# CYF2000127/MolNexTR

Hardware: AMD Instinct MI355X
Metric: molecules/sec (384x384, bs32 per GPU), full predict hot path (higher is better)
Workload: dtype fp16x3

## Files before the change

include/molnextr_hip.h:

```cpp
#ifndef MOLNEXTR_HIP_H
#define MOLNEXTR_HIP_H

#include <stddef.h>
#include <stdint.h>

#ifdef __cplusplus
extern "C" {
#endif

#define MNX_ABI_VERSION 7

typedef struct mnx_engine mnx_engine;

typedef enum {
    MNX_OK = 0,
    MNX_ERR_INVALID_ARG = -1,
    MNX_ERR_WEIGHTS = -2,
    MNX_ERR_HIP = -3,
    MNX_ERR_NO_DEVICE = -4,
    MNX_ERR_CAPACITY = -5,
    MNX_ERR_RANGE = -6
} mnx_status;

enum { MNX_DTYPE_BF16 = 0, MNX_DTYPE_FP16 = 1, MNX_DTYPE_FP32 = 2, MNX_DTYPE_BF16X3 = 3, MNX_DTYPE_FP16X3 = 4,
// ... 177 lines not shown
               int32_t N, int32_t K, void* stream);

int mnx_gemm16_split(mnx_engine* h, int32_t epi, const void* A, int64_t a_lo, const void* W, int64_t w_lo, float oscale,
                     void* C, int64_t c_lo, const float* bias, int32_t M, int32_t N, int32_t K, int32_t terms,
                     void* stream);

int mnx_window_attn(mnx_engine* h, const void* qkv, int64_t qkv_lo, const float* table, void* out, int64_t out_lo,
                    int32_t B, int32_t H, int32_t W, int32_t C, int32_t heads, int32_t shift, int32_t terms, void* stream);

int mnx_kv_block(mnx_engine* h, int32_t which, int32_t layer, int32_t owner, int32_t head, void* dst, void* stream);

int mnx_patch_embed(mnx_engine* h, const void* img, int32_t img_format, const float* w_t, const float* bias,
                    const float* gamma, const float* beta, float* x, int32_t B, int32_t S, int32_t C, void* stream);

int mnx_layernorm16(mnx_engine* h, const float* x, const float* gamma, const float* beta, void* y16, int64_t y_lo,
                    float* y32, int32_t M, int32_t C, float eps, int32_t planes, int32_t* flag, void* stream);
int mnx_merge_ln16(mnx_engine* h, const float* x, const float* gamma, const float* beta, void* y16, int64_t y_lo,
                   int32_t B, int32_t H, int32_t W, int32_t C, float eps, int32_t planes, void* stream);

int mnx_cast16(mnx_engine* h, const float* x, void* y16, int64_t y_lo, int64_t n, float scale, void* stream);

int mnx_sgemm_tn(mnx_engine* h, const float* A, const float* W, const float* bias, float* C, int32_t M, int32_t N,
                 int32_t K, int32_t perm_S, void* stream);

int mnx_profile_enable(mnx_engine* h, int32_t enable);
int mnx_profile_read(mnx_engine* h, int32_t kind, double* ms, double* work, int64_t* launches);

int mnx_probe_decode_attn(mnx_engine* h, int32_t rows, int32_t t, int32_t iters, double* self_ms, double* cross_ms,
                          void* stream);

int mnx_gemm_clock(mnx_engine* h, int32_t reset, double* mhz);
int mnx_probe_mfma(mnx_engine* h, int32_t ms_target, double* tflops, double* mhz, void* stream);

#ifdef __cplusplus
}
#endif
#endif
```

molnextr_amd/csrc/atom_walk.h:

```cpp
#pragma once
#include "dec_types.h"

namespace mnx {

template <typename Emit>
__device__ __forceinline__ int atom_walk(const int* seq, int n, const unsigned char* fl, const TokenClasses* __restrict__ tc,
                                         Emit emit) {
    const int x0 = tc->x0, y0 = tc->y0, lb = tc->lbracket, rb = tc->rbracket;
    const int iC = tc->id_C, il = tc->id_l, iB = tc->id_B, ir = tc->id_r;
    int i = 0, k = 0;
    while (i < n) {
        const int t = seq[i];
        if (t == 2 || t == 0) break;
        if (t >= x0) { ++i; continue; }
        if (!(fl[t] & 2)) { ++i; continue; }
        int j;
        if (t == lb) {
            j = i + 1;
            while (j < n && seq[j] < x0 && (fl[seq[j]] & 1)) {
                ++j;
                if (seq[j - 1] == rb) break;
            }
        } else if (i + 1 < n && ((t == iC && seq[i + 1] == il) || (t == iB && seq[i + 1] == ir))) {
            j = i + 2;
        } else {
            j = i + 1;
        }
        if (j + 2 < n && seq[j] >= x0 && seq[j] < y0 && seq[j + 1] >= y0) {
            emit(k, i, j);
            ++k;
            i = j + 2;
        } else {
            i = j;
        }
    }
    return k;
}

}
```

molnextr_amd/csrc/dec_types.h:

```cpp
#pragma once
#include <hip/hip_runtime.h>
#include <stdint.h>

struct mnx_mol;
struct mnx_atom;
struct mnx_bond;
struct mnx_molfile;
struct mnx_smiles;

namespace mnx {

constexpr int MAX_SLOTS = 4096;
constexpr int BEGIN_THREADS = 1024;
constexpr int ROW_TILE = 32;
constexpr int MAX_DEC_LAYERS = 8;
constexpr int MAX_CHUNKS = 128;
constexpr int MAX_REF_BATCH = 512;
constexpr int CHUNK_TILES = MAX_REF_BATCH / ROW_TILE;

struct DecState {
    int tick;
    int n_active;
    int chunk_alive[MAX_CHUNKS];
    int alive[MAX_SLOTS];
// ... 21 lines not shown
    const float *lnf_g, *lnf_b;
    const float *w1, *b1, *w2, *b2;
    const float *wqkv_t, *wo_t, *wq2_t, *wo2_t, *w1_t, *w2_t;
};

struct DecWeights {
    DecLayerW L[MAX_DEC_LAYERS];
    const float *emb, *pe, *lnF_g, *lnF_b, *wout_t, *bout;
    const float *w_enc, *b_enc;
    const float *w_memkv, *b_memkv;
    const float *edge_w1cat, *edge_b1cat;
    const float *edge_w2, *edge_b2;
    int layers, heads, dff, vocab, vpad, sym_offset, bins, pe_len, enc_dim;
};

struct DecBuffers {
    DecState* st;
    float *x, *q, *ctx, *h;
    float *x2, *part;
    float *fpart;
    int fpart_rows;
    char *self_k, *self_v;
    float *memory;
    float *mem_kv32;
    char *mem_kv;
    int Tq, Sq;
    int* tokens;
    float* logp;
    float* hidden;
    float *edge_g, *edge_uv, *edge_prob;
    int T, S, slots, mem_blocks, kmax;
};

constexpr int MAX_BEAM_IMGS = 256;
constexpr int MAX_BEAM = 8;
constexpr int BEAM_LP_STRIDE = 256;
constexpr int BEAM_ANC_MAX = 512;

struct BeamState {
    int top_fin[MAX_BEAM_IMGS];
    int n_hyps[MAX_BEAM_IMGS];
    int pool_n[MAX_BEAM_IMGS];
    int order[MAX_BEAM_IMGS][MAX_BEAM];
    float pscore[MAX_BEAM_IMGS][MAX_BEAM];
    int plen[MAX_BEAM_IMGS][MAX_BEAM];
    float cum[MAX_BEAM_IMGS * MAX_BEAM];
};

struct BeamBuffers {
    BeamState* bs;
    float* blp;
    int* anc;
    int* ptok;
    float* phid;
    int B, K, n_best, anc_stride;
    int ref_batch;
    int pool_stride;
};

struct TokenClasses {
    unsigned char flags[256];
    int lbracket, rbracket, id_C, id_l, id_B, id_r, x0, y0, vocab;
};

struct VocabText {
    unsigned char len[256];
    unsigned char name[256][8];
};

hipError_t kvq_pack_enqueue(const float* src, char* dst, int n_blocks, int S, int Sq, hipStream_t s);
constexpr int GUIDE_MASK = 4;
struct GuideRows {
    int* table;
    int stride;
    const int* src;
    int L, n;
};
hipError_t dec_enqueue_admit(const DecBuffers& b, const int* slots_dev, const int* rowc_dev, int n, int chunk_tag,
                             int mem_blk0, int max_len, int stop_on_eos, hipStream_t s, const GuideRows* g = nullptr);
hipError_t dec_enqueue_reset(const DecBuffers& b, hipStream_t s);
hipError_t dec_enqueue_status(const DecBuffers& b, int slots, hipStream_t s);
hipError_t dec_enqueue_tick(const DecWeights& w, const DecBuffers& b, int slots_scan, int rows, float* logits_trace,
                            int trace_rows, hipStream_t s, const BeamBuffers* beam = nullptr, const int* forced = nullptr,
                            int fused_tile = 0, const int* glab = nullptr, int glab_stride = 0);
hipError_t dec_fused_init();
void dec_fused_dump_stamps(const char* path);
hipError_t dec_enqueue_fused_layers(const DecWeights& w, const DecBuffers& b, int rows, int row_tile, hipStream_t s,
                                    const float** x_final, const float** part_final);
hipError_t beam_enqueue_init(const DecBuffers& b, const BeamBuffers& bm, int max_len, hipStream_t s);
hipError_t beam_enqueue_gather(const DecBuffers& b, const BeamBuffers& bm, int out_len, int* o_tokens, int* o_len,
                               float* o_scores, float* o_hidden, hipStream_t s);
hipError_t dec_probe_attn(const DecWeights& w, const DecBuffers& b, int rows, int t, int iters, hipEvent_t* ev,
                          hipStream_t s);
// ... 39 lines not shown
```

molnextr_amd/csrc/decoder.hip:

```cpp
#include <stdlib.h>

#include "common.h"
#include "kernels.h"
#include "dec_types.h"
#include "atom_walk.h"
#include "kvq.h"

namespace mnx {

__global__ __launch_bounds__(256) void sgemm_tn_kernel(const float* __restrict__ A, const float* __restrict__ W,
                                                       const float* __restrict__ bias, float* __restrict__ C, int M,
                                                       int N, int K, int perm_S) {
    __shared__ float As[16][68], Ws[16][68];
    const int tid = threadIdx.x, tx = tid & 15, ty = tid >> 4;
    const int m0 = blockIdx.y * 64, n0 = blockIdx.x * 64;
    const int lr = tid >> 2, lk = (tid & 3) * 4;
    const float* ap = A + (size_t)min(m0 + lr, M - 1) * K + lk;
    const float* wp = W + (size_t)min(n0 + lr, N - 1) * K + lk;
    float acc[4][4] = {};
    f32x4 a = *(const f32x4*)ap, w = *(const f32x4*)wp;
    for (int k0 = 0; k0 < K; k0 += 16) {
#pragma unroll
        for (int j = 0; j < 4; ++j) {
            As[lk + j][lr] = a[j];
            Ws[lk + j][lr] = w[j];
        }
        __syncthreads();
        const int kn = k0 + 16 < K ? k0 + 16 : k0;
// ... 5 lines not shown
#pragma unroll
            for (int i = 0; i < 4; ++i)
#pragma unroll
                for (int j = 0; j < 4; ++j) acc[i][j] = fmaf(av[i], wv[j], acc[i][j]);
        }
        __syncthreads();
    }
    const int n = n0 + tx * 4;
    if (n >= N) return;
    f32x4 b4 = {0.f, 0.f, 0.f, 0.f};
    if (bias) b4 = *(const f32x4*)(bias + n);
#pragma unroll
    for (int i = 0; i < 4; ++i) {
        const int m = m0 + ty * 4 + i;
        if (m < M) {
            const size_t off = perm_S > 0 ? ((((size_t)(m / perm_S) * (N >> 8) + (n >> 8)) * 8 + ((n & 255) >> 5)) * perm_S +
                                             (m % perm_S)) * 32 + (n & 31)
                                          : (size_t)m * N + n;
            *(f32x4*)(C + off) = (f32x4){acc[i][0], acc[i][1], acc[i][2], acc[i][3]} + b4;
        }
    }
}

hipError_t launch_sgemm_tn(const float* A, const float* W, const float* bias, float* C, int M, int N, int K,
                           hipStream_t s, int perm_S) {
    if ((K & 15) || (N & 3) || (perm_S > 0 && ((N & 255) || M % perm_S))) return hipErrorInvalidValue;
    dim3 grid((N + 63) / 64, (M + 63) / 64), block(256);
    hipLaunchKernelGGL(sgemm_tn_kernel, grid, block, 0, s, A, W, bias, C, M, N, K, perm_S);
    return hipGetLastError();
}

__global__ __launch_bounds__(256) void kvq_pack_kernel(const float* __restrict__ src, char* __restrict__ dst, long long n_rows,
                                                       int S, int Sq) {
    const long long r = (long long)blockIdx.x * 32 + (threadIdx.x >> 3);
    const int part = threadIdx.x & 7;
    if (r >= n_rows) return;
    const f32x4 v = *(const f32x4*)(src + r * 32 + part * 4);
    float amax = fmaxf(fmaxf(fabsf(v[0]), fabsf(v[1])), fmaxf(fabsf(v[2]), fabsf(v[3])));
    amax = fmaxf(amax, __shfl_xor(amax, 1, 64));
    amax = fmaxf(amax, __shfl_xor(amax, 2, 64));
    amax = fmaxf(amax, __shfl_xor(amax, 4, 64));
    int q[4];
    float scale = 0.f;
#pragma unroll
    for (int u = 0; u < 4; ++u) kvq_quant(v[u], amax, q[u], scale);
    const long long blk_i = r / S;
    const int key = (int)(r - blk_i * S);
    char* blk = dst + (size_t)blk_i * kvq_block_bytes(Sq);
    kvq_store4(blk, Sq, key, part * 4, q);
    if (part == 0) kvq_store_scale(blk, Sq, key, scale);
}

hipError_t kvq_pack_enqueue(const float* src, char* dst, int n_blocks, int S, int Sq, hipStream_t s) {
    const long long n_rows = (long long)n_blocks * S;
    hipLaunchKernelGGL(kvq_pack_kernel, dim3((unsigned)((n_rows + 31) / 32)), dim3(256), 0, s, src, dst, n_rows, S, Sq);
    return hipGetLastError();
}


constexpr int TN = 32, XS = 260;

struct LinArgs {
    const float* in;
    const float* W;
    const float* bias;
    const float* gamma;
    const float* beta;
    float* out;
    char* kcache;
    char* vcache;
    int Tq;
    float* x_write;
    const float* emb;
    const float* pe;
    const float* part;
    const DecState* st;
    int N, K, T, heads;
    int part_stride;
// ... 498 lines not shown
    h.x = (split_w2 && ((w.layers - 1) & 1)) ? b.x2 : b.x; h.part = split_w2 ? b.part : nullptr; h.part_stride = b.slots * D;
    h.n_part = w.dff / 256;
    if (fused) { h.x = fx; h.part = fp; h.part_stride = b.fpart_rows * D; h.tree_bias = w.L[w.layers - 1].b2; }
    h.gamma = w.lnF_g; h.beta = w.lnF_b; h.wout_t = w.wout_t; h.bout = w.bout; h.st = b.st;
    h.tokens = b.tokens; h.token_logp = b.logp; h.hidden = b.hidden; h.logits_trace = logits_trace;
    h.V = w.vocab; h.VP = w.vpad; h.T = T; h.x0 = w.sym_offset; h.y0 = w.sym_offset + w.bins;
    h.eos = 2; h.trace_rows = trace_rows; h.forced = forced;
    const GuideTab gt{glab, glab_stride};
    if (glab) {
        if (fused) hipLaunchKernelGGL(dec_head4_guided_kernel, dim3(slots), dim3(1024), 0, s, h, gt);
        else hipLaunchKernelGGL(dec_head_guided_kernel, dim3(slots), dim3(256), 0, s, h, gt);
    } else if (beam) {
        h.blp = beam->blp;
        hipLaunchKernelGGL(dec_head_kernel<true>, dim3(slots), dim3(256), 0, s, h);
        hipLaunchKernelGGL(beam_pick_kernel, dim3(beam->B), dim3(256), 0, s, b.st, *beam, b.hidden, b.tokens, T, w.vocab, 2);
    } else if (fused) {
        hipLaunchKernelGGL(dec_head4_kernel, dim3(slots), dim3(1024), 0, s, h);
    } else {
        hipLaunchKernelGGL(dec_head_kernel<false>, dim3(slots), dim3(256), 0, s, h);
    }
    return hipGetLastError();
}

__global__ __launch_bounds__(64) void atom_scan_kernel(const int* __restrict__ lens, const int* __restrict__ tokens,
                                                       const TokenClasses* __restrict__ tc, const int* __restrict__ slots,
                                                       int n_rows, int T, int kmax, int* __restrict__ atom_idx,
                                                       int* __restrict__ n_atoms) {
    __shared__ int seq[512];
    __shared__ unsigned char fl[256];
    const int row = blockIdx.x;
    const int slot = slots ? slots[row] : row;
    const int n = min(lens[slot], 512);
    for (int i = threadIdx.x; i < n; i += 64) seq[i] = tokens[(size_t)slot * T + i];
    for (int i = threadIdx.x; i < 256; i += 64) fl[i] = tc->flags[i];
    __syncthreads();
    if (threadIdx.x != 0) return;
    const int k = atom_walk(seq, n, fl, tc, [&](int a, int, int j) {
        if (a < kmax) atom_idx[(size_t)row * kmax + a] = j + 2;
    });
    n_atoms[row] = k < kmax ? k : kmax;
}

hipError_t atoms_enqueue(const DecBuffers& b, const TokenClasses* tc_dev, const int* slots_dev, int n, int kmax,
                         int* atom_idx, int* n_atoms, hipStream_t s) {
    hipLaunchKernelGGL(atom_scan_kernel, dim3(n), dim3(64), 0, s, b.st->len, b.tokens, tc_dev, slots_dev, n, b.T, kmax,
                       atom_idx, n_atoms);
    return hipGetLastError();
}

hipError_t atoms_enqueue_raw(const TokenClasses* tc_dev, const int* tokens, const int* lens, int n, int T, int kmax,
                             int* atom_idx, int* n_atoms, hipStream_t s) {
    hipLaunchKernelGGL(atom_scan_kernel, dim3(n), dim3(64), 0, s, lens, tokens, tc_dev, (const int*)nullptr, n, T, kmax,
                       atom_idx, n_atoms);
    return hipGetLastError();
}

constexpr int CONF_THREADS = 256;

__global__ __launch_bounds__(CONF_THREADS) void confidence_kernel(
        const int* __restrict__ lens, const int* __restrict__ tokens, const float* __restrict__ logp,
        const TokenClasses* __restrict__ tc, const int* __restrict__ slots, int T, int kmax,
        const int* __restrict__ atom_idx, const int* __restrict__ n_atoms, const double* __restrict__ scores,
        double* __restrict__ atom_scores, double* __restrict__ overall) {
    __shared__ int seq[512];
    __shared__ double ts[512];
    __shared__ unsigned char fl[256];
    __shared__ int span_len[256];
    __shared__ double red_sum[CONF_THREADS], red_prod[CONF_THREADS];
    const int row = blockIdx.x, tid = threadIdx.x;
    const int slot = slots ? slots[row] : row;
    const int n = min(min(lens[slot], T), 512);
    const int k = min(max(n_atoms[row], 0), kmax);
    double sum = 0.0, prod = 1.0;
    for (int i = tid; i < n; i += CONF_THREADS) {
        seq[i] = tokens[(size_t)slot * T + i];
// ... 443 lines not shown
```

molnextr_amd/csrc/engine.hip:

```cpp
#include "../../include/molnextr_hip.h"

#include <hip/hip_runtime.h>

#include <time.h>
#include <cmath>
#include <cstdint>
#include <cstdio>
#include <cstring>
#include <map>
#include <memory>
#include <string>
#include <tuple>
#include <unordered_map>
#include <vector>

#include "dec_types.h"
#include "kernels.h"
#include "kvq.h"

using namespace mnx;

namespace {

thread_local std::string g_create_error;
// ... 516 lines not shown
    if (h->enc_flag && hipMemset(h->enc_flag, 0, sizeof(int)) != hipSuccess) P.problems.push_back("hipMemset failed");
    DecBuffers& db = h->db;
    const int SL = c.dec_slots > 0 ? c.dec_slots : 2048;
    h->n_chunk_bufs = SL / ROW_TILE;
    db.T = c.max_len; db.S = (int)S; db.slots = SL; db.mem_blocks = h->n_chunk_bufs * ROW_TILE; db.kmax = c.max_atoms;
    db.st = (DecState*)P.dalloc(sizeof(DecState));
    db.x = (float*)P.dalloc((size_t)SL * D * 4);
    db.x2 = (float*)P.dalloc((size_t)SL * D * 4);
    db.part = (float*)P.dalloc((size_t)(FF / 256) * SL * D * 4);
    db.fpart_rows = std::min(SL, std::max(ROW_TILE, (std::max(h->dec_fused_max, h->dec_mid_max) + ROW_TILE - 1) / ROW_TILE * ROW_TILE));
    db.fpart = (float*)P.dalloc((size_t)2 * 16 * db.fpart_rows * D * 4);
    if (db.fpart && hipMemset(db.fpart, 0, (size_t)2 * 16 * db.fpart_rows * D * 4) != hipSuccess) P.problems.push_back("hipMemset failed");
    if (dec_fused_init() != hipSuccess) P.problems.push_back("dec_fused_init: LDS opt-in failed");
    db.q = (float*)P.dalloc((size_t)SL * D * 4);
    db.ctx = (float*)P.dalloc((size_t)SL * D * 4);
    db.h = (float*)P.dalloc((size_t)SL * FF * 4);
    db.Tq = kvq_rows(c.max_len); db.Sq = kvq_rows((int)S);
    const size_t cache = (size_t)c.dec_layers * SL * c.dec_heads * kvq_block_bytes(db.Tq);
    db.self_k = (char*)P.dalloc(cache);
    db.self_v = (char*)P.dalloc(cache);
    if (db.self_k && db.self_v && (hipMemset(db.self_k, 0, cache) != hipSuccess || hipMemset(db.self_v, 0, cache) != hipSuccess))
        P.problems.push_back("hipMemset failed");
    db.memory = (float*)P.dalloc((size_t)ROW_TILE * S * D * 4);
    db.mem_kv32 = (float*)P.dalloc((size_t)ROW_TILE * S * c.dec_layers * 2 * D * 4);
    const size_t mem_bytes = (size_t)db.mem_blocks * c.dec_layers * 2 * c.dec_heads * kvq_block_bytes(db.Sq);
    db.mem_kv = (char*)P.dalloc(mem_bytes);
    if (db.mem_kv && hipMemset(db.mem_kv, 0, mem_bytes) != hipSuccess) P.problems.push_back("hipMemset failed");
    db.tokens = (int*)P.dalloc((size_t)SL * c.max_len * 4);
    db.logp = (float*)P.dalloc((size_t)SL * c.max_len * 4);
    db.hidden = (float*)P.dalloc((size_t)SL * c.max_len * D * 4);
    db.edge_g = (float*)P.dalloc((size_t)ROW_TILE * db.kmax * D * 4);
    db.edge_uv = (float*)P.dalloc((size_t)ROW_TILE * db.kmax * 2 * D * 4);
    db.edge_prob = (float*)P.dalloc((size_t)ROW_TILE * db.kmax * db.kmax * 8 * 4);
    const size_t ring_rows = std::max<size_t>(ROW_TILE, MB);
    h->feat_ring[0] = (float*)P.dalloc(ring_rows * S * CF * 4);
    h->feat_ring[1] = (float*)P.dalloc(ring_rows * S * CF * 4);
    h->slot_lists = (int*)P.dalloc((size_t)MAX_CHUNKS * ROW_TILE * 4);
    h->rowc_seq = (int*)P.dalloc((size_t)MAX_REF_BATCH * 4);
    if (h->rowc_seq) {
        std::vector<int> seq_rows(MAX_REF_BATCH);
        for (int i = 0; i < MAX_REF_BATCH; ++i) seq_rows[i] = i;
        if (hipMemcpy(h->rowc_seq, seq_rows.data(), (size_t)MAX_REF_BATCH * 4, hipMemcpyHostToDevice) != hipSuccess)
            P.problems.push_back("row index table upload failed");
    }
    h->tc_dev = (TokenClasses*)P.dalloc(sizeof(TokenClasses));
    h->vt_dev = (VocabText*)P.dalloc(sizeof(VocabText));
    h->st_dev = (SymbolTables*)P.dalloc(sizeof(SymbolTables));
// ... 204 lines not shown
    HIPCHK(h, hipSetDevice(h->device));
    *s = (hipStream_t)stream;
    if (!*s) {
        if (!h->own_stream) HIPCHK(h, hipStreamCreate(&h->own_stream));
        *s = h->own_stream;
    }
    return MNX_OK;
}

template <typename T>
int lazy_alloc(mnx_engine* h, T** p, size_t bytes) {
    if (*p) return MNX_OK;
    HIPCHK(h, hipMalloc((void**)p, bytes));
    h->allocs.push_back(*p);
    h->bytes += bytes;
    return MNX_OK;
}

int project_memory(mnx_engine* h, const float* feats, int n, int blk0, hipStream_t s) {
    const mnx_config& c = h->cfg;
    const int S = h->db.S, D = c.dec_dim;
    char* memkv = h->db.mem_kv + (size_t)blk0 * c.dec_layers * 2 * c.dec_heads * kvq_block_bytes(h->db.Sq);
    HIPCHK(h, launch_sgemm_tn(feats, h->dw.w_enc, h->dw.b_enc, h->db.memory, n * S, D, h->dw.enc_dim, s));
    HIPCHK(h, launch_sgemm_tn(h->db.memory, h->dw.w_memkv, h->dw.b_memkv, h->db.mem_kv32, n * S, c.dec_layers * 2 * D, D, s, S));
    HIPCHK(h, kvq_pack_enqueue(h->db.mem_kv32, memkv, n * c.dec_layers * 2 * c.dec_heads, S, h->db.Sq, s));
    return MNX_OK;
}

struct FeatRing {
    mnx_engine* h;
    const void* images;
    int fmt;
    int n_img, ref_batch, n_chunks, grp;
    int first[2] = {-1, -1}, count[2] = {0, 0};
    bool used[2] = {false, false};
    int next_enc = 0;

    int refill() {
        const size_t img_bytes = (size_t)h->cfg.img_size * h->cfg.img_size * (fmt == MNX_IMG_GRAY8 ? 1 : 3 * sizeof(float));
        for (int i = 0; i < 2; ++i) {
            if (first[i] >= 0 || next_enc >= n_chunks) continue;
            const int cnt = std::min(grp, n_chunks - next_enc);
            const int f = next_enc * ref_batch, n = std::min(cnt * ref_batch, n_img - f);
            if (used[i]) HIPCHK(h, hipStreamWaitEvent(h->enc_stream, h->ev_feat_free[i], 0));
            MNXCHK(encode_impl(h, fmt == MNX_IMG_GRAY8 ? "mnx_encode_gray8" : "mnx_encode", (const char*)images + (size_t)f * img_bytes,
                               fmt, n, h->feat_ring[i], h->enc_stream));
            HIPCHK(h, hipEventRecord(h->ev_enc_done[i], h->enc_stream));
            first[i] = next_enc;
// ... 951 lines not shown
    HIPCHK(h, hipSetDevice(h->device));
    HIPCHK(h, launch_merge_ln16(h->dt, x, gamma, beta, y16, B, H, W, C, eps, (hipStream_t)stream, (size_t)y_lo, planes));
    return MNX_OK;
}

int mnx_cast16(mnx_engine* h, const float* x, void* y16, int64_t y_lo, int64_t n, float scale, void* stream) {
    if (!h) return MNX_ERR_INVALID_ARG;
    auto bad = [&](const char* m) { h->err = std::string("mnx_cast16: ") + m; return MNX_ERR_INVALID_ARG; };
    if (!x || !y16) return bad("null pointer");
    if (((uintptr_t)x & 15) || ((uintptr_t)y16 & 7) || (h->dt == MNX_DT_F32 && ((uintptr_t)y16 & 15)))
        return bad("x must be 16-byte aligned, y16 8-byte (16-byte for FP32)");
    if (n < 4 || (n & 3)) return bad("n must be a positive multiple of 4");
    if (dt_split(h->dt)) {
        if (y_lo < n || (y_lo & 3)) return bad("y_lo must be at least n and a multiple of 4 elements");
        if (!(scale > 0.f) || !(scale < INFINITY)) return bad("scale must be positive and finite");
    } else if (y_lo) {
        return bad("y_lo must be 0 for the single-plane compute_dtypes");
    }
    HIPCHK(h, hipSetDevice(h->device));
    HIPCHK(h, launch_cast16(h->dt, x, y16, (size_t)n, (hipStream_t)stream, (size_t)y_lo, scale));
    return MNX_OK;
}

int mnx_sgemm_tn(mnx_engine* h, const float* A, const float* W, const float* bias, float* C, int32_t M, int32_t N,
                 int32_t K, int32_t perm_S, void* stream) {
    if (!h) return MNX_ERR_INVALID_ARG;
    auto bad = [&](const char* m) { h->err = std::string("mnx_sgemm_tn: ") + m; return MNX_ERR_INVALID_ARG; };
    if (!A || !W || !C) return bad("null pointer");
    if (misaligned16({A, W, bias, C})) return bad("A, W, bias and C must be 16-byte aligned");
    if (M < 1 || N < 4 || K < 16) return bad("M >= 1, N >= 4 and K >= 16 required");
    if (K & 15) return bad("K must be a multiple of 16");
    if (N & 3) return bad("N must be a multiple of 4");
    if (perm_S < 0) return bad("perm_S must not be negative");
    if (perm_S > 0 && (N & 255)) return bad("perm_S needs N to be a multiple of 256");
    if (perm_S > 0 && M % perm_S) return bad("perm_S must divide M");
    if ((M + 63) / 64 > 65535) return bad("M must be at most 65535 * 64");
    HIPCHK(h, hipSetDevice(h->device));
    HIPCHK(h, launch_sgemm_tn(A, W, bias, C, M, N, K, (hipStream_t)stream, perm_S));
    return MNX_OK;
}

}
```

molnextr_amd/csrc/kernels.h:

```cpp
#pragma once
#include <hip/hip_runtime.h>
#include <stdint.h>

#include "../../include/molnextr_hip.h"

namespace mnx {

enum { MNX_DT_BF16 = 0, MNX_DT_F16 = 1, MNX_DT_F32 = 2, MNX_DT_BF16X3 = 3, MNX_DT_F16X3 = 4 };
inline bool dt_split(int dtype) { return dtype == MNX_DT_BF16X3 || dtype == MNX_DT_F16X3; }
inline int dt_base(int dtype) { return dtype == MNX_DT_BF16X3 ? MNX_DT_BF16 : dtype == MNX_DT_F16X3 ? MNX_DT_F16 : dtype; }
inline size_t dt_size(int dtype) { return (dtype == MNX_DT_F32 || dt_split(dtype)) ? 4 : 2; }
enum { EPI_BIAS_16 = 0, EPI_GELU_16 = 1, EPI_RESID_F32 = 2, EPI_BIAS_F32 = 3 };

struct SplitArgs {
    size_t a_lo = 0, w_lo = 0, c_lo = 0;
    float oscale = 1.f;
    int terms = 3;
    int c_planes = 2;
};

hipError_t launch_gemm16(int dtype, int epi, const void* A, const void* W, void* C, const float* bias,
                         const float* resid, int M, int N, int K, hipStream_t s, const SplitArgs* sp = nullptr);
const char* gemm16_route(int dtype, int epi, int M, int N, int K, int terms, bool has_bias);
hipError_t launch_gemm16_tile128(int dtype, int epi, const void* A, const void* W, void* C, const float* bias,
// ... 18 lines not shown
                              const float* beta, float* x, int B, int S, int C, hipStream_t s);
hipError_t launch_patch_embed_gray8(const uint8_t* gray, const float* w_t , const float* bias, const float* gamma,
                                    const float* beta, float* x, int B, int S, int C, hipStream_t s);
hipError_t launch_layernorm16(int dtype, const float* x, const float* gamma, const float* beta, void* y16, float* y32,
                              int M, int C, float eps, hipStream_t s, size_t y_lo = 0, int* nonfinite_flag = nullptr,
                              int planes = 2);
hipError_t launch_merge_ln16(int dtype, const float* x, const float* gamma, const float* beta, void* y16, int B, int H,
                             int W, int C, float eps, hipStream_t s, size_t y_lo = 0, int planes = 2);
hipError_t launch_window_attn(int dtype, const void* qkv16, const float* rel_table, void* out16, int B, int H, int W,
                              int C, int heads, int shift, hipStream_t s, size_t qkv_lo = 0, size_t out_lo = 0,
                              int terms = 3);
hipError_t launch_cast16(int dtype, const float* x, void* y16, size_t n, hipStream_t s, size_t y_lo = 0,
                         float scale = 1.f);

hipError_t launch_preprocess(const uint8_t* rgb, int H, int W, int pad, int square, int S, int* bbox, int* crop_out,
                             float* out, hipStream_t s);
struct NormConsts { float mean255[3], inv[3]; };
NormConsts norm_consts();
hipError_t launch_preprocess_batch(const uint8_t* arena, const mnx_page* pages, int n, int max_height, int pad, int square,
                                   int S, int* bbox, int* crops, void* out, bool gray8, hipStream_t s);

struct DecWeights;
struct DecState;
hipError_t launch_sgemm_tn(const float* A, const float* W, const float* bias, float* C, int M, int N, int K,
                           hipStream_t s, int perm_S = 0);

}
```

molnextr_amd/engine.py:

```python
from __future__ import annotations

import ctypes as C
import os
from typing import Dict, Optional

import numpy as np
import torch

from . import weights as W

_LIB_PATH = os.path.join(os.path.dirname(os.path.abspath(__file__)), "lib", "libmolnextr_hip.so")
_lib = None

ABI_VERSION = 7
SYMBOLS = ("mnx_abi_version", "mnx_create", "mnx_destroy", "mnx_last_error", "mnx_workspace_bytes", "mnx_encode",
           "mnx_set_encoder_tap", "mnx_decode_greedy", "mnx_edges", "mnx_gemm16", "mnx_profile_enable",
           "mnx_profile_read", "mnx_set_token_classes", "mnx_predict", "mnx_atom_scan", "mnx_decode_beam", "mnx_preprocess",
           "mnx_probe_decode_attn", "mnx_predict_beam", "mnx_set_split_terms", "mnx_encoder_status",
           "mnx_gemm16_split", "mnx_decode_forced", "mnx_gemm_clock", "mnx_probe_mfma", "mnx_set_op_terms",
           "mnx_predict_confidence", "mnx_confidence", "mnx_window_attn", "mnx_kv_block", "mnx_preprocess_batch",
           "mnx_encode_gray8", "mnx_predict_gray8", "mnx_decode_guided", "mnx_predict_guided", "mnx_patch_embed",
           "mnx_layernorm16", "mnx_merge_ln16", "mnx_cast16", "mnx_sgemm_tn", "mnx_set_vocab_text", "mnx_graph_pack",
           "mnx_set_symbol_tables", "mnx_molfile_pack", "mnx_smiles_pack")

DTYPES = {"bf16": 0, "fp16": 1, "fp32": 2, "bf16x3": 3, "fp16x3": 4, "fp16x3m": 5}
DEFAULT_DTYPE = "fp16x3"
SPLIT_CLASSES = {"qkv": 1, "attn": 2, "proj": 4, "fc1": 8, "fc2": 16, "merge": 32}
FP16X3M_BLOCKS = {}
FP16X3M_TWO_TERM = ("qkv.s2", "fc1.s2", "fc2.s2")


def two_term_masks(two_term, n_stages):
    masks = [0] * n_stages
    for tag in two_term:
        cls, _, st = tag.partition(".s")
        for i in ([int(st)] if st else range(n_stages)):
            masks[i] |= SPLIT_CLASSES[cls]
    return masks


class MnxConfig(C.Structure):
    _fields_ = [("img_size", C.c_int32), ("patch", C.c_int32), ("embed_dim", C.c_int32), ("n_stages", C.c_int32),
                ("depths", C.c_int32 * 4), ("heads", C.c_int32 * 4), ("window", C.c_int32),
                ("dec_layers", C.c_int32), ("dec_dim", C.c_int32), ("dec_heads", C.c_int32), ("dec_ff", C.c_int32),
                ("vocab", C.c_int32), ("sym_offset", C.c_int32), ("coord_bins", C.c_int32), ("pe_len", C.c_int32),
                ("max_len", C.c_int32), ("max_batch", C.c_int32), ("max_atoms", C.c_int32),
# ... 121 lines not shown
    lib.mnx_decode_greedy.argtypes = [vp, vp, i32, vp, i32, i32, vp, vp, vp, vp, vp, vp]
    lib.mnx_decode_forced.restype = C.c_int
    lib.mnx_decode_forced.argtypes = [vp, vp, i32, vp, i32, vp, vp, vp, vp, vp, vp]
    lib.mnx_edges.restype = C.c_int
    lib.mnx_edges.argtypes = [vp, vp, vp, vp, i32, i32, i32, vp, vp, vp]
    lib.mnx_gemm16.restype = C.c_int
    lib.mnx_gemm16.argtypes = [vp, i32, vp, vp, vp, vp, i32, i32, i32, vp]
    lib.mnx_gemm16_split.restype = C.c_int
    lib.mnx_gemm16_split.argtypes = [vp, i32, vp, C.c_int64, vp, C.c_int64, C.c_float, vp, C.c_int64, vp, i32, i32, i32, i32, vp]
    lib.mnx_window_attn.restype = C.c_int
    lib.mnx_window_attn.argtypes = [vp, vp, C.c_int64, vp, vp, C.c_int64, i32, i32, i32, i32, i32, i32, i32, vp]
    lib.mnx_kv_block.restype = C.c_int
    lib.mnx_kv_block.argtypes = [vp, i32, i32, i32, i32, vp, vp]
    lib.mnx_patch_embed.restype = C.c_int
    lib.mnx_patch_embed.argtypes = [vp, vp, i32, vp, vp, vp, vp, vp, i32, i32, i32, vp]
    lib.mnx_layernorm16.restype = C.c_int
    lib.mnx_layernorm16.argtypes = [vp, vp, vp, vp, vp, C.c_int64, vp, i32, i32, C.c_float, i32, vp, vp]
    lib.mnx_merge_ln16.restype = C.c_int
    lib.mnx_merge_ln16.argtypes = [vp, vp, vp, vp, vp, C.c_int64, i32, i32, i32, i32, C.c_float, i32, vp]
    lib.mnx_cast16.restype = C.c_int
    lib.mnx_cast16.argtypes = [vp, vp, vp, C.c_int64, C.c_int64, C.c_float, vp]
    lib.mnx_sgemm_tn.restype = C.c_int
    lib.mnx_sgemm_tn.argtypes = [vp, vp, vp, vp, vp, i32, i32, i32, i32, vp]
    lib.mnx_profile_enable.restype = C.c_int
    lib.mnx_profile_enable.argtypes = [vp, i32]
    lib.mnx_profile_read.restype = C.c_int
    lib.mnx_profile_read.argtypes = [vp, i32, C.POINTER(C.c_double), C.POINTER(C.c_double), C.POINTER(C.c_int64)]
    lib.mnx_probe_decode_attn.restype = C.c_int
    lib.mnx_probe_decode_attn.argtypes = [vp, i32, i32, i32, C.POINTER(C.c_double), C.POINTER(C.c_double), vp]
    lib.mnx_gemm_clock.restype = C.c_int
    lib.mnx_gemm_clock.argtypes = [vp, i32, C.POINTER(C.c_double)]
    lib.mnx_probe_mfma.restype = C.c_int
    lib.mnx_probe_mfma.argtypes = [vp, i32, C.POINTER(C.c_double), C.POINTER(C.c_double), vp]
    lib.mnx_set_token_classes.restype = C.c_int
    lib.mnx_set_token_classes.argtypes = [vp, C.c_char_p, i32, i32, i32, i32, i32, i32, i32]
    lib.mnx_set_vocab_text.restype = C.c_int
    lib.mnx_set_vocab_text.argtypes = [vp, C.c_char_p, vp, i32]
    lib.mnx_graph_pack.restype = C.c_int
    lib.mnx_graph_pack.argtypes = [vp, vp, vp, i32, i32, vp, vp, vp, i32, vp, vp, vp, vp, vp, C.c_uint32, vp, C.c_uint32, vp,
                                   C.c_uint32, vp, vp]
    lib.mnx_set_symbol_tables.restype = C.c_int
    lib.mnx_set_symbol_tables.argtypes = [vp, C.c_char_p, vp, vp, i32]
    lib.mnx_molfile_pack.restype = C.c_int
    lib.mnx_molfile_pack.argtypes = [vp, vp, i32, vp, C.c_uint32, vp, C.c_uint32, vp, C.c_uint32, vp, vp, vp, C.c_uint32, vp, vp]
    lib.mnx_smiles_pack.restype = C.c_int
    lib.mnx_smiles_pack.argtypes = [vp, vp, i32, vp, C.c_uint32, vp, C.c_uint32, vp, C.c_uint32, vp, vp, vp, C.c_uint32, vp, vp]
# ... 658 lines not shown
        self._check(self.lib.mnx_patch_embed(self.h, _ptr(img), fmt, _ptr(w_t), _ptr(bias), _ptr(gamma), _ptr(beta), _ptr(x),
                                             B, S, C_, _stream()), "mnx_patch_embed")
        return x

    def layernorm16(self, x: torch.Tensor, gamma: torch.Tensor, beta: torch.Tensor, y16: Optional[torch.Tensor],
                    y32: Optional[torch.Tensor], M: int, C_: int, eps: float = 1e-5, y_lo: int = 0, planes: int = 2,
                    flag: Optional[torch.Tensor] = None):
        self._check(self.lib.mnx_layernorm16(self.h, _ptr(x), _ptr(gamma), _ptr(beta), _ptr(y16), y_lo, _ptr(y32), M, C_,
                                             float(eps), planes, _ptr(flag), _stream()), "mnx_layernorm16")

    def merge_ln16(self, x: torch.Tensor, gamma: torch.Tensor, beta: torch.Tensor, y16: torch.Tensor, B: int, H: int,
                   W_: int, C_: int, eps: float = 1e-5, y_lo: int = 0, planes: int = 2):
        self._check(self.lib.mnx_merge_ln16(self.h, _ptr(x), _ptr(gamma), _ptr(beta), _ptr(y16), y_lo, B, H, W_, C_,
                                            float(eps), planes, _stream()), "mnx_merge_ln16")

    def cast16(self, x: torch.Tensor, y16: torch.Tensor, n: int, y_lo: int = 0, scale: float = 1.0):
        self._check(self.lib.mnx_cast16(self.h, _ptr(x), _ptr(y16), y_lo, n, float(scale), _stream()), "mnx_cast16")

    def sgemm_tn(self, A: torch.Tensor, Wt: torch.Tensor, bias: Optional[torch.Tensor], Cout: torch.Tensor, M: int, N: int,
                 K: int, perm_S: int = 0):
        self._check(self.lib.mnx_sgemm_tn(self.h, _ptr(A), _ptr(Wt), _ptr(bias), _ptr(Cout), M, N, K, perm_S, _stream()),
                    "mnx_sgemm_tn")

    def gemm16(self, epi: int, A: torch.Tensor, Wt: torch.Tensor, Cout: torch.Tensor, bias: Optional[torch.Tensor]):
        M, K = A.shape
        N = Wt.shape[0]
        self._check(self.lib.mnx_gemm16(self.h, epi, _ptr(A), _ptr(Wt), _ptr(Cout), _ptr(bias), M, N, K, _stream()),
                    "mnx_gemm16")
        return Cout
```

Measured before the change: 2184.

## Use MFMA fp32 sgemm, fuse KV quant into GEMM, parallelize atom scan

Swaps the scalar fp32 sgemm_tn for a double-buffered MFMA 32x32x1 f32 kernel with 128-row tiles and a wider variant for large grids. The memory K/V projection now quantizes and packs kvq blocks in the GEMM epilogue, which removes the fp32 staging buffer and the separate pack kernel. The per-row atom scan, formerly one serial thread, now uses 512 threads: each computes its step, pointer jumping marks reachable positions, and a block scan assigns indices. This adds complexity and changes the GEMM accumulation order, and the old kernel is kept as a reference entry point.

Result: no change. 2198 (median of 6 runs) (+0.6%).

```diff
diff --git a/include/molnextr_hip.h b/include/molnextr_hip.h
--- a/include/molnextr_hip.h
+++ b/include/molnextr_hip.h
@@ -223,6 +223,8 @@
 
 int mnx_sgemm_tn(mnx_engine* h, const float* A, const float* W, const float* bias, float* C, int32_t M, int32_t N,
                  int32_t K, int32_t perm_S, void* stream);
+int mnx_sgemm_tn_ref(mnx_engine* h, const float* A, const float* W, const float* bias, float* C, int32_t M, int32_t N,
+                     int32_t K, int32_t perm_S, void* stream);
 
 int mnx_profile_enable(mnx_engine* h, int32_t enable);
 int mnx_profile_read(mnx_engine* h, int32_t kind, double* ms, double* work, int64_t* launches);
diff --git a/molnextr_amd/csrc/atom_walk.h b/molnextr_amd/csrc/atom_walk.h
--- a/molnextr_amd/csrc/atom_walk.h
+++ b/molnextr_amd/csrc/atom_walk.h
@@ -3,36 +3,51 @@
 
 namespace mnx {
 
+struct AtomWalkIds { int x0, y0, lb, rb, iC, il, iB, ir; };
+__device__ __forceinline__ AtomWalkIds atom_walk_ids(const TokenClasses* __restrict__ tc) {
+    return {tc->x0, tc->y0, tc->lbracket, tc->rbracket, tc->id_C, tc->id_l, tc->id_B, tc->id_r};
+}
+__device__ __forceinline__ int atom_step(const int* seq, int n, const unsigned char* fl, const AtomWalkIds& c, int i, int* j_out,
+                                         bool* atom) {
+    *atom = false;
+    const int t = seq[i];
+    if (t == 2 || t == 0) return n;
+    if (t >= c.x0) return i + 1;
+    if (!(fl[t] & 2)) return i + 1;
+    int j;
+    if (t == c.lb) {
+        j = i + 1;
+        while (j < n && seq[j] < c.x0 && (fl[seq[j]] & 1)) {
+            ++j;
+            if (seq[j - 1] == c.rb) break;
+        }
+    } else if (i + 1 < n && ((t == c.iC && seq[i + 1] == c.il) || (t == c.iB && seq[i + 1] == c.ir))) {
+        j = i + 2;
+    } else {
+        j = i + 1;
+    }
+    if (j + 2 < n && seq[j] >= c.x0 && seq[j] < c.y0 && seq[j + 1] >= c.y0) {
+        *j_out = j;
+        *atom = true;
+        return j + 2;
+    }
+    return j;
+}
+
 template <typename Emit>
 __device__ __forceinline__ int atom_walk(const int* seq, int n, const unsigned char* fl, const TokenClasses* __restrict__ tc,
                                          Emit emit) {
-    const int x0 = tc->x0, y0 = tc->y0, lb = tc->lbracket, rb = tc->rbracket;
-    const int iC = tc->id_C, il = tc->id_l, iB = tc->id_B, ir = tc->id_r;
+    const AtomWalkIds c = atom_walk_ids(tc);
     int i = 0, k = 0;
     while (i < n) {
-        const int t = seq[i];
-        if (t == 2 || t == 0) break;
-        if (t >= x0) { ++i; continue; }
-        if (!(fl[t] & 2)) { ++i; continue; }
-        int j;
-        if (t == lb) {
-            j = i + 1;
-            while (j < n && seq[j] < x0 && (fl[seq[j]] & 1)) {
-                ++j;
-                if (seq[j - 1] == rb) break;
-            }
-        } else if (i + 1 < n && ((t == iC && seq[i + 1] == il) || (t == iB && seq[i + 1] == ir))) {
-            j = i + 2;
-        } else {
-            j = i + 1;
-        }
-        if (j + 2 < n && seq[j] >= x0 && seq[j] < y0 && seq[j + 1] >= y0) {
+        int j = 0;
+        bool atom;
+        const int next = atom_step(seq, n, fl, c, i, &j, &atom);
+        if (atom) {
             emit(k, i, j);
             ++k;
-            i = j + 2;
-        } else {
-            i = j;
         }
+        i = next;
     }
     return k;
 }
diff --git a/molnextr_amd/csrc/dec_types.h b/molnextr_amd/csrc/dec_types.h
--- a/molnextr_amd/csrc/dec_types.h
+++ b/molnextr_amd/csrc/dec_types.h
@@ -67,7 +67,6 @@
     int fpart_rows;
     char *self_k, *self_v;
     float *memory;
-    float *mem_kv32;
     char *mem_kv;
     int Tq, Sq;
     int* tokens;
@@ -113,7 +112,6 @@
     unsigned char name[256][8];
 };
 
-hipError_t kvq_pack_enqueue(const float* src, char* dst, int n_blocks, int S, int Sq, hipStream_t s);
 constexpr int GUIDE_MASK = 4;
 struct GuideRows {
     int* table;
diff --git a/molnextr_amd/csrc/decoder.hip b/molnextr_amd/csrc/decoder.hip
--- a/molnextr_amd/csrc/decoder.hip
+++ b/molnextr_amd/csrc/decoder.hip
@@ -4,6 +4,7 @@
 #include "kernels.h"
 #include "dec_types.h"
 #include "atom_walk.h"
+#include "block_scan.h"
 #include "kvq.h"
 
 namespace mnx {
@@ -55,38 +56,11 @@
     }
 }
 
-hipError_t launch_sgemm_tn(const float* A, const float* W, const float* bias, float* C, int M, int N, int K,
-                           hipStream_t s, int perm_S) {
+hipError_t launch_sgemm_tn_ref(const float* A, const float* W, const float* bias, float* C, int M, int N, int K,
+                               hipStream_t s, int perm_S) {
     if ((K & 15) || (N & 3) || (perm_S > 0 && ((N & 255) || M % perm_S))) return hipErrorInvalidValue;
     dim3 grid((N + 63) / 64, (M + 63) / 64), block(256);
     hipLaunchKernelGGL(sgemm_tn_kernel, grid, block, 0, s, A, W, bias, C, M, N, K, perm_S);
-    return hipGetLastError();
-}
-
-__global__ __launch_bounds__(256) void kvq_pack_kernel(const float* __restrict__ src, char* __restrict__ dst, long long n_rows,
-                                                       int S, int Sq) {
-    const long long r = (long long)blockIdx.x * 32 + (threadIdx.x >> 3);
-    const int part = threadIdx.x & 7;
-    if (r >= n_rows) return;
-    const f32x4 v = *(const f32x4*)(src + r * 32 + part * 4);
-    float amax = fmaxf(fmaxf(fabsf(v[0]), fabsf(v[1])), fmaxf(fabsf(v[2]), fabsf(v[3])));
-    amax = fmaxf(amax, __shfl_xor(amax, 1, 64));
-    amax = fmaxf(amax, __shfl_xor(amax, 2, 64));
-    amax = fmaxf(amax, __shfl_xor(amax, 4, 64));
-    int q[4];
-    float scale = 0.f;
-#pragma unroll
-    for (int u = 0; u < 4; ++u) kvq_quant(v[u], amax, q[u], scale);
-    const long long blk_i = r / S;
-    const int key = (int)(r - blk_i * S);
-    char* blk = dst + (size_t)blk_i * kvq_block_bytes(Sq);
-    kvq_store4(blk, Sq, key, part * 4, q);
-    if (part == 0) kvq_store_scale(blk, Sq, key, scale);
-}
-
-hipError_t kvq_pack_enqueue(const float* src, char* dst, int n_blocks, int S, int Sq, hipStream_t s) {
-    const long long n_rows = (long long)n_blocks * S;
-    hipLaunchKernelGGL(kvq_pack_kernel, dim3((unsigned)((n_rows + 31) / 32)), dim3(256), 0, s, src, dst, n_rows, S, Sq);
     return hipGetLastError();
 }
 
@@ -631,35 +605,54 @@
     return hipGetLastError();
 }
 
-__global__ __launch_bounds__(64) void atom_scan_kernel(const int* __restrict__ lens, const int* __restrict__ tokens,
-                                                       const TokenClasses* __restrict__ tc, const int* __restrict__ slots,
-                                                       int n_rows, int T, int kmax, int* __restrict__ atom_idx,
-                                                       int* __restrict__ n_atoms) {
-    __shared__ int seq[512];
+constexpr int SCAN_THREADS = 512;
+
+__global__ __launch_bounds__(SCAN_THREADS) void atom_scan_kernel(const int* __restrict__ lens, const int* __restrict__ tokens,
+                                                                 const TokenClasses* __restrict__ tc,
+                                                                 const int* __restrict__ slots, int n_rows, int T, int kmax,
+                                                                 int* __restrict__ atom_idx, int* __restrict__ n_atoms) {
+    __shared__ int seq[SCAN_THREADS];
     __shared__ unsigned char fl[256];
-    const int row = blockIdx.x;
+    __shared__ int nxt[SCAN_THREADS + 1];
+    __shared__ int seen[SCAN_THREADS + 1];
+    __shared__ unsigned scan[2 * SCAN_THREADS];
+    const int row = blockIdx.x, tid = threadIdx.x;
     const int slot = slots ? slots[row] : row;
-    const int n = min(lens[slot], 512);
-    for (int i = threadIdx.x; i < n; i += 64) seq[i] = tokens[(size_t)slot * T + i];
-    for (int i = threadIdx.x; i < 256; i += 64) fl[i] = tc->flags[i];
-    __syncthreads();
-    if (threadIdx.x != 0) return;
-    const int k = atom_walk(seq, n, fl, tc, [&](int a, int, int j) {
-        if (a < kmax) atom_idx[(size_t)row * kmax + a] = j + 2;
-    });
-    n_atoms[row] = k < kmax ? k : kmax;
+    const int n = max(min(lens[slot], SCAN_THREADS), 0);
+    if (tid < n) seq[tid] = tokens[(size_t)slot * T + tid];
+    if (tid < 256) fl[tid] = tc->flags[tid];
+    __syncthreads();
+    int j = 0;
+    bool atom = false;
+    nxt[tid] = tid < n ? atom_step(seq, n, fl, atom_walk_ids(tc), tid, &j, &atom) : n;
+    seen[tid] = tid == 0;
+    if (tid == 0) { nxt[n] = n; seen[SCAN_THREADS] = 0; }
+    __syncthreads();
+    for (int d = 1; d <= n; d <<= 1) {
+        const int to = nxt[tid], to2 = nxt[to];
+        const bool mark = seen[tid] != 0;
+        __syncthreads();
+        if (mark) seen[to] = 1;
+        nxt[tid] = to2;
+        __syncthreads();
+    }
+    const bool found = atom && seen[tid] != 0;
+    unsigned total;
+    const unsigned a = block_scan_excl<SCAN_THREADS>(found ? 1u : 0u, scan, &total);
+    if (found && (int)a < kmax) atom_idx[(size_t)row * kmax + a] = j + 2;
+    if (tid == 0) n_atoms[row] = (int)total < kmax ? (int)total : kmax;
 }
 
 hipError_t atoms_enqueue(const DecBuffers& b, const TokenClasses* tc_dev, const int* slots_dev, int n, int kmax,
                          int* atom_idx, int* n_atoms, hipStream_t s) {
-    hipLaunchKernelGGL(atom_scan_kernel, dim3(n), dim3(64), 0, s, b.st->len, b.tokens, tc_dev, slots_dev, n, b.T, kmax,
+    hipLaunchKernelGGL(atom_scan_kernel, dim3(n), dim3(SCAN_THREADS), 0, s, b.st->len, b.tokens, tc_dev, slots_dev, n, b.T, kmax,
                        atom_idx, n_atoms);
     return hipGetLastError();
 }
 
 hipError_t atoms_enqueue_raw(const TokenClasses* tc_dev, const int* tokens, const int* lens, int n, int T, int kmax,
                              int* atom_idx, int* n_atoms, hipStream_t s) {
-    hipLaunchKernelGGL(atom_scan_kernel, dim3(n), dim3(64), 0, s, lens, tokens, tc_dev, (const int*)nullptr, n, T, kmax,
+    hipLaunchKernelGGL(atom_scan_kernel, dim3(n), dim3(SCAN_THREADS), 0, s, lens, tokens, tc_dev, (const int*)nullptr, n, T, kmax,
                        atom_idx, n_atoms);
     return hipGetLastError();
 }
diff --git a/molnextr_amd/csrc/engine.hip b/molnextr_amd/csrc/engine.hip
--- a/molnextr_amd/csrc/engine.hip
+++ b/molnextr_amd/csrc/engine.hip
@@ -562,7 +562,6 @@
     if (db.self_k && db.self_v && (hipMemset(db.self_k, 0, cache) != hipSuccess || hipMemset(db.self_v, 0, cache) != hipSuccess))
         P.problems.push_back("hipMemset failed");
     db.memory = (float*)P.dalloc((size_t)ROW_TILE * S * D * 4);
-    db.mem_kv32 = (float*)P.dalloc((size_t)ROW_TILE * S * c.dec_layers * 2 * D * 4);
     const size_t mem_bytes = (size_t)db.mem_blocks * c.dec_layers * 2 * c.dec_heads * kvq_block_bytes(db.Sq);
     db.mem_kv = (char*)P.dalloc(mem_bytes);
     if (db.mem_kv && hipMemset(db.mem_kv, 0, mem_bytes) != hipSuccess) P.problems.push_back("hipMemset failed");
@@ -813,8 +812,7 @@
     const int S = h->db.S, D = c.dec_dim;
     char* memkv = h->db.mem_kv + (size_t)blk0 * c.dec_layers * 2 * c.dec_heads * kvq_block_bytes(h->db.Sq);
     HIPCHK(h, launch_sgemm_tn(feats, h->dw.w_enc, h->dw.b_enc, h->db.memory, n * S, D, h->dw.enc_dim, s));
-    HIPCHK(h, launch_sgemm_tn(h->db.memory, h->dw.w_memkv, h->dw.b_memkv, h->db.mem_kv32, n * S, c.dec_layers * 2 * D, D, s, S));
-    HIPCHK(h, kvq_pack_enqueue(h->db.mem_kv32, memkv, n * c.dec_layers * 2 * c.dec_heads, S, h->db.Sq, s));
+    HIPCHK(h, launch_sgemm_tn_kvq(h->db.memory, h->dw.w_memkv, h->dw.b_memkv, memkv, n * S, c.dec_layers * 2 * D, D, S, h->db.Sq, s));
     return MNX_OK;
 }
 
@@ -1812,10 +1810,10 @@
     return MNX_OK;
 }
 
-int mnx_sgemm_tn(mnx_engine* h, const float* A, const float* W, const float* bias, float* C, int32_t M, int32_t N,
-                 int32_t K, int32_t perm_S, void* stream) {
-    if (!h) return MNX_ERR_INVALID_ARG;
-    auto bad = [&](const char* m) { h->err = std::string("mnx_sgemm_tn: ") + m; return MNX_ERR_INVALID_ARG; };
+static int sgemm_tn_aid(mnx_engine* h, const char* name, bool ref, const float* A, const float* W, const float* bias, float* C,
+                        int32_t M, int32_t N, int32_t K, int32_t perm_S, void* stream) {
+    if (!h) return MNX_ERR_INVALID_ARG;
+    auto bad = [&](const char* m) { h->err = std::string(name) + ": " + m; return MNX_ERR_INVALID_ARG; };
     if (!A || !W || !C) return bad("null pointer");
     if (misaligned16({A, W, bias, C})) return bad("A, W, bias and C must be 16-byte aligned");
     if (M < 1 || N < 4 || K < 16) return bad("M >= 1, N >= 4 and K >= 16 required");
@@ -1826,8 +1824,18 @@
     if (perm_S > 0 && M % perm_S) return bad("perm_S must divide M");
     if ((M + 63) / 64 > 65535) return bad("M must be at most 65535 * 64");
     HIPCHK(h, hipSetDevice(h->device));
-    HIPCHK(h, launch_sgemm_tn(A, W, bias, C, M, N, K, (hipStream_t)stream, perm_S));
-    return MNX_OK;
-}
-
-}
+    HIPCHK(h, (ref ? launch_sgemm_tn_ref : launch_sgemm_tn)(A, W, bias, C, M, N, K, (hipStream_t)stream, perm_S));
+    return MNX_OK;
+}
+
+int mnx_sgemm_tn(mnx_engine* h, const float* A, const float* W, const float* bias, float* C, int32_t M, int32_t N,
+                 int32_t K, int32_t perm_S, void* stream) {
+    return sgemm_tn_aid(h, "mnx_sgemm_tn", false, A, W, bias, C, M, N, K, perm_S, stream);
+}
+
+int mnx_sgemm_tn_ref(mnx_engine* h, const float* A, const float* W, const float* bias, float* C, int32_t M, int32_t N,
+                     int32_t K, int32_t perm_S, void* stream) {
+    return sgemm_tn_aid(h, "mnx_sgemm_tn_ref", true, A, W, bias, C, M, N, K, perm_S, stream);
+}
+
+}
diff --git a/molnextr_amd/csrc/kernels.h b/molnextr_amd/csrc/kernels.h
--- a/molnextr_amd/csrc/kernels.h
+++ b/molnextr_amd/csrc/kernels.h
@@ -64,7 +64,12 @@
 
 struct DecWeights;
 struct DecState;
+hipError_t launch_sgemm_tn_ref(const float* A, const float* W, const float* bias, float* C, int M, int N, int K,
+                               hipStream_t s, int perm_S = 0);
+
 hipError_t launch_sgemm_tn(const float* A, const float* W, const float* bias, float* C, int M, int N, int K,
                            hipStream_t s, int perm_S = 0);
+hipError_t launch_sgemm_tn_kvq(const float* A, const float* W, const float* bias, char* blocks, int M, int N, int K, int S,
+                               int Sq, hipStream_t s);
 
 }
diff --git a/molnextr_amd/csrc/sgemm.hip b/molnextr_amd/csrc/sgemm.hip
--- /dev/null
+++ b/molnextr_amd/csrc/sgemm.hip
@@ -0,0 +1,145 @@
+#include "common.h"
+#include "kernels.h"
+#include "dec_types.h"
+#include "kvq.h"
+
+namespace mnx {
+
+namespace {
+
+typedef float f32x32 __attribute__((ext_vector_type(32)));
+constexpr int SG_KS = 16, SG_LD = SG_KS + 4, SG_BM = 128;
+
+template <int RW, bool QUANT>
+__global__ __launch_bounds__(256) void sgemm_mfma_kernel(const float* __restrict__ A, const float* __restrict__ W,
+                                                         const float* __restrict__ bias, float* __restrict__ C,
+                                                         char* __restrict__ blocks, int M, int N, int K, int perm_S, int Sq) {
+    constexpr int BM = SG_BM, BN = 64 * RW, Q = SG_KS / 4;
+    constexpr int LA = BM * Q / 256, LW = BN * Q / 256;
+    __shared__ __attribute__((aligned(16))) float As[2][BM][SG_LD];
+    __shared__ __attribute__((aligned(16))) float Ws[2][BN][SG_LD];
+    const int tid = threadIdx.x, lane = tid & 63, wave = tid >> 6, wm = wave & 1, wn = wave >> 1;
+    const int m0 = blockIdx.y * BM, n0 = blockIdx.x * BN;
+    const int lk = (tid % Q) * 4;
+    const float* ap[LA];
+    const float* wp[LW];
+    f32x4 a[LA], w[LW];
+#pragma unroll
+    for (int u = 0; u < LA; ++u) ap[u] = A + (size_t)min(m0 + (tid + u * 256) / Q, M - 1) * K + lk;
+#pragma unroll
+    for (int u = 0; u < LW; ++u) wp[u] = W + (size_t)min(n0 + (tid + u * 256) / Q, N - 1) * K + lk;
+    auto fetch = [&](int k0) {
+#pragma unroll
+        for (int u = 0; u < LA; ++u) a[u] = *(const f32x4*)(ap[u] + k0);
+#pragma unroll
+        for (int u = 0; u < LW; ++u) w[u] = *(const f32x4*)(wp[u] + k0);
+    };
+    auto stage = [&](int buf) {
+#pragma unroll
+        for (int u = 0; u < LA; ++u) *(f32x4*)&As[buf][(tid + u * 256) / Q][lk] = a[u];
+#pragma unroll
+        for (int u = 0; u < LW; ++u) *(f32x4*)&Ws[buf][(tid + u * 256) / Q][lk] = w[u];
+    };
+    f32x32 acc[RW];
+#pragma unroll
+    for (int r = 0; r < RW; ++r)
+#pragma unroll
+        for (int v = 0; v < 32; ++v) acc[r][v] = 0.f;
+    fetch(0);
+    stage(0);
+    __syncthreads();
+    int buf = 0;
+    for (int k0 = 0; k0 < K; k0 += SG_KS) {
+        const bool more = k0 + SG_KS < K;
+        if (more) fetch(k0 + SG_KS);
+#pragma unroll
+        for (int kq = 0; kq < Q; ++kq) {
+            const f32x4 av = *(const f32x4*)&As[buf][wm * 64 + lane][kq * 4];
+            f32x4 wv[RW];
+#pragma unroll
+            for (int r = 0; r < RW; ++r) wv[r] = *(const f32x4*)&Ws[buf][(wn * RW + r) * 32 + (lane & 31)][kq * 4];
+#pragma unroll
+            for (int kk = 0; kk < 4; ++kk)
+#pragma unroll
+                for (int r = 0; r < RW; ++r) acc[r] = __builtin_amdgcn_mfma_f32_32x32x1f32(wv[r][kk], av[kk], acc[r], 0, 0, 0);
+        }
+        if (more) stage(buf ^ 1);
+        __syncthreads();
+        buf ^= 1;
+    }
+#pragma unroll
+    for (int r = 0; r < RW; ++r) {
+        const int nb = n0 + (wn * RW + r) * 32;
+#pragma unroll
+        for (int bl = 0; bl < 2; ++bl) {
+            const int m = m0 + wm * 64 + bl * 32 + (lane & 31);
+            f32x4 v[4];
+#pragma unroll
+            for (int g = 0; g < 4; ++g) {
+                const int n = nb + g * 8 + (lane >> 5) * 4;
+                f32x4 b4 = {0.f, 0.f, 0.f, 0.f};
+                if (bias && n < N) b4 = *(const f32x4*)(bias + n);
+                v[g] = (f32x4){acc[r][bl * 16 + g * 4], acc[r][bl * 16 + g * 4 + 1], acc[r][bl * 16 + g * 4 + 2],
+                               acc[r][bl * 16 + g * 4 + 3]} + b4;
+            }
+            if (QUANT) {
+                float amax = 0.f;
+#pragma unroll
+                for (int g = 0; g < 4; ++g)
+                    amax = fmaxf(amax, fmaxf(fmaxf(fabsf(v[g][0]), fabsf(v[g][1])), fmaxf(fabsf(v[g][2]), fabsf(v[g][3]))));
+                amax = fmaxf(amax, __shfl_xor(amax, 32, 64));
+                const int img = m / perm_S, key = m - img * perm_S;
+                const size_t blk_i = ((size_t)img * (N >> 8) + (nb >> 8)) * 8 + ((nb & 255) >> 5);
+                char* blk = blocks + blk_i * kvq_block_bytes(Sq);
+                float scale = 0.f;
+#pragma unroll
+                for (int g = 0; g < 4; ++g) {
+                    int q[4];
+#pragma unroll
+                    for (int u = 0; u < 4; ++u) kvq_quant(v[g][u], amax, q[u], scale);
+                    if (m < M) kvq_store4(blk, Sq, key, g * 8 + (lane >> 5) * 4, q);
+                }
+                if (m < M && lane < 32) kvq_store_scale(blk, Sq, key, scale);
+            } else if (m < M) {
+#pragma unroll
+                for (int g = 0; g < 4; ++g) {
+                    const int n = nb + g * 8 + (lane >> 5) * 4;
+                    if (n >= N) continue;
+                    const size_t off = perm_S > 0 ? ((((size_t)(m / perm_S) * (N >> 8) + (n >> 8)) * 8 + ((n & 255) >> 5)) * perm_S +
+                                                     (m % perm_S)) * 32 + (n & 31)
+                                                  : (size_t)m * N + n;
+                    *(f32x4*)(C + off) = v[g];
+                }
+            }
+        }
+    }
+}
+
+template <bool QUANT>
+hipError_t sgemm_dispatch(const float* A, const float* W, const float* bias, float* C, char* blocks, int M, int N, int K,
+                          hipStream_t s, int perm_S, int Sq) {
+    const int mt = (M + SG_BM - 1) / SG_BM;
+    if ((long long)mt * ((N + 127) / 128) >= 256)
+        hipLaunchKernelGGL((sgemm_mfma_kernel<2, QUANT>), dim3((N + 127) / 128, mt), dim3(256), 0, s, A, W, bias, C, blocks, M, N,
+                           K, perm_S, Sq);
+    else
+        hipLaunchKernelGGL((sgemm_mfma_kernel<1, QUANT>), dim3((N + 63) / 64, mt), dim3(256), 0, s, A, W, bias, C, blocks, M, N,
+                           K, perm_S, Sq);
+    return hipGetLastError();
+}
+
+}
+
+hipError_t launch_sgemm_tn(const float* A, const float* W, const float* bias, float* C, int M, int N, int K,
+                           hipStream_t s, int perm_S) {
+    if ((K & 15) || (N & 3) || (perm_S > 0 && ((N & 255) || M % perm_S))) return hipErrorInvalidValue;
+    return sgemm_dispatch<false>(A, W, bias, C, nullptr, M, N, K, s, perm_S, 0);
+}
+
+hipError_t launch_sgemm_tn_kvq(const float* A, const float* W, const float* bias, char* blocks, int M, int N, int K, int S,
+                               int Sq, hipStream_t s) {
+    if ((K & 15) || (N & 255) || S < 1 || M % S || Sq < S) return hipErrorInvalidValue;
+    return sgemm_dispatch<true>(A, W, bias, nullptr, blocks, M, N, K, s, S, Sq);
+}
+
+}
diff --git a/molnextr_amd/engine.py b/molnextr_amd/engine.py
--- a/molnextr_amd/engine.py
+++ b/molnextr_amd/engine.py
@@ -21,7 +21,7 @@
            "mnx_predict_confidence", "mnx_confidence", "mnx_window_attn", "mnx_kv_block", "mnx_preprocess_batch",
            "mnx_encode_gray8", "mnx_predict_gray8", "mnx_decode_guided", "mnx_predict_guided", "mnx_patch_embed",
            "mnx_layernorm16", "mnx_merge_ln16", "mnx_cast16", "mnx_sgemm_tn", "mnx_set_vocab_text", "mnx_graph_pack",
-           "mnx_set_symbol_tables", "mnx_molfile_pack", "mnx_smiles_pack")
+           "mnx_set_symbol_tables", "mnx_molfile_pack", "mnx_smiles_pack", "mnx_sgemm_tn_ref")
 
 DTYPES = {"bf16": 0, "fp16": 1, "fp32": 2, "bf16x3": 3, "fp16x3": 4, "fp16x3m": 5}
 DEFAULT_DTYPE = "fp16x3"
@@ -189,6 +189,8 @@
     lib.mnx_cast16.argtypes = [vp, vp, vp, C.c_int64, C.c_int64, C.c_float, vp]
     lib.mnx_sgemm_tn.restype = C.c_int
     lib.mnx_sgemm_tn.argtypes = [vp, vp, vp, vp, vp, i32, i32, i32, i32, vp]
+    lib.mnx_sgemm_tn_ref.restype = C.c_int
+    lib.mnx_sgemm_tn_ref.argtypes = [vp, vp, vp, vp, vp, i32, i32, i32, i32, vp]
     lib.mnx_profile_enable.restype = C.c_int
     lib.mnx_profile_enable.argtypes = [vp, i32]
     lib.mnx_profile_read.restype = C.c_int
@@ -893,6 +895,11 @@
         self._check(self.lib.mnx_sgemm_tn(self.h, _ptr(A), _ptr(Wt), _ptr(bias), _ptr(Cout), M, N, K, perm_S, _stream()),
                     "mnx_sgemm_tn")
 
+    def sgemm_tn_ref(self, A: torch.Tensor, Wt: torch.Tensor, bias: Optional[torch.Tensor], Cout: torch.Tensor, M: int, N: int,
+                     K: int, perm_S: int = 0):
+        self._check(self.lib.mnx_sgemm_tn_ref(self.h, _ptr(A), _ptr(Wt), _ptr(bias), _ptr(Cout), M, N, K, perm_S, _stream()),
+                    "mnx_sgemm_tn_ref")
+
     def gemm16(self, epi: int, A: torch.Tensor, Wt: torch.Tensor, Cout: torch.Tensor, bias: Optional[torch.Tensor]):
         M, K = A.shape
         N = Wt.shape[0]
```
